# LPD-EPFL-ML/X-MAP

Measured on AMD Instinct MI355X. Metric: item_sim_pairs_per_s, higher is better.
Workload: dtype f64

## Files before the change

x-map_amd/csrc/api.hip:

```cpp
#include <math.h>
#include <stdlib.h>
#include <vector>

#include "common.h"

namespace xmap {

struct Pool {
    std::vector<void *> ptrs;
    void release() {
        for (void *p : ptrs) (void)hipFree(p);
        ptrs.clear();
    }
};

}

using namespace xmap;

struct xmap_ctx {
    int device = 0;
    hipStream_t st = nullptr;
    Pool p_ratings, p_sim, p_ext, p_gen, p_rows;
    xmap_ratings R;
    bool have_ratings = false;
    bool plain_exact = true;
    bool have_sim = false;
    xmap_sim S;
    double *u_avg = nullptr, *u_norm = nullptr, *info = nullptr;
    int64_t n_kept = 0, n_eval = 0, n_contrib = 0;
    int64_t half_contrib = 0;
    bool have_ext = false;
    int top_k = 0;
    xmap_ext_tables T;
    xmap_path_units Un;
    int32_t *n_cand = nullptr, *top_end = nullptr;
    double *top_val = nullptr;
    int64_t n_out = 0, n_paths = 0;
    double *acc = nullptr, *hacc = nullptr;
    int32_t *touched = nullptr, *htouched = nullptr;
    int64_t acc_slots = 0, acc_len = 0, hacc_rows = 0, hacc_len = 0;
    int32_t n_slots = 0;
    int32_t fast_div = 0;
    bool have_gen = false;
    int32_t *g_user = nullptr, *g_item = nullptr;
    double *g_rating = nullptr;
    int64_t *g_time = nullptr;
    int64_t n_rows = 0, n_target_rows = 0;
};

namespace xmap {

template <typename T>
static int dalloc(Pool &pool, T **out, size_t n, hipStream_t st, bool zero = false) {
    void *p = nullptr;
    const size_t bytes = sizeof(T) * (n ? n : 1);
    XM_HIP(hipMalloc(&p, bytes));
    pool.ptrs.push_back(p);
    if (zero) XM_HIP(hipMemsetAsync(p, 0, bytes, st));
    *out = (T *)p;
    return XMAP_OK;
}
#define XM_TRY(call) do { int rc_ = (call); if (rc_) return rc_; } while (0)
#define XM_ALLOC(pool, ptr, n) XM_TRY(dalloc(pool, &(ptr), (size_t)(n), c->st))
#define XM_ALLOCZ(pool, ptr, n) XM_TRY(dalloc(pool, &(ptr), (size_t)(n), c->st, true))

template <typename T>
static int h2d(Pool &pool, T **out, const T *host, size_t n, hipStream_t st) {
    XM_TRY(dalloc(pool, out, n, st));
    if (n) XM_HIP(hipMemcpyAsync(*out, host, sizeof(T) * n, hipMemcpyHostToDevice, st));
    return XMAP_OK;
}
template <typename T>
static int d2h(T *host, const T *dev, size_t n, hipStream_t st) {
    if (n) XM_HIP(hipMemcpyAsync(host, dev, sizeof(T) * n, hipMemcpyDeviceToHost, st));
    return XMAP_OK;
}

static int reverse_list(xmap_ctx *c, int mode, const uint8_t *bb, const int64_t *attach_ptr, const void *thr, int32_t *long_rows,
                        uint8_t *eflag, int32_t *counted ,
                        const int64_t **rptr, const int32_t **ridx, const double **rval, const uint8_t **rflag) {
    const int I = c->R.n_items, k = c->top_k;
    int32_t *rcnt = counted;
    int64_t *ptr;
    XM_ALLOCZ(c->p_ext, ptr, I + 1);
    if (!counted) {
        XM_ALLOCZ(c->p_ext, rcnt, I);
        XM_TRY(xmap_reverse_count(c->st, &c->S, mode, k, bb, c->T.cls, c->T.kcnt, c->T.kcol, c->T.kval, c->R.suffix_cls,
                                  c->R.contains_mask, c->R.flags, attach_ptr, thr, long_rows, eflag, rcnt, 0, I));
    }
    int64_t n = 0;
    XM_TRY(xmap_exclusive_scan_i32_to_i64(c->st, rcnt, ptr, I, &n));
    int32_t *idx;
    double *val;
    uint8_t *flag;
    XM_ALLOC(c->p_ext, idx, n);
    XM_ALLOC(c->p_ext, val, 3 * (size_t)(n ? n : 1));
    XM_ALLOCZ(c->p_ext, flag, n);
    XM_TRY(xmap_reverse_fill(c->st, &c->S, mode, k, bb, c->T.cls, c->T.kcnt, c->T.kcol, c->T.kval, c->R.suffix_cls,
                             c->R.contains_mask, c->R.flags, attach_ptr, thr, long_rows, eflag, ptr, idx, val, flag, 0, I));
    *rptr = ptr; *ridx = idx; *rval = val; *rflag = flag;
    return XMAP_OK;
}

static int ensure_rows(xmap_ctx *c, int64_t slots, int64_t len, int64_t hrows) {
    if (c->acc == nullptr || c->acc_slots < slots || c->acc_len != len || c->hacc_rows < hrows) {
        c->p_rows.release();
        c->acc = nullptr; c->hacc = nullptr;
        XM_ALLOCZ(c->p_rows, c->acc, (size_t)slots * len * 4);
        XM_ALLOC(c->p_rows, c->touched, (size_t)slots * len);
        if (hrows) {
            XM_ALLOCZ(c->p_rows, c->hacc, (size_t)hrows * len * 4);
            XM_ALLOC(c->p_rows, c->htouched, (size_t)hrows * len);
        }
        c->acc_slots = slots; c->acc_len = len; c->hacc_rows = hrows;
    }
    return XMAP_OK;
}

static int run_enumeration(xmap_ctx *c, int64_t xs_cap, int64_t *xs_off, int32_t *xs_end, double *xs_val) {
    const int I = c->R.n_items;
    xmap_path_rows Rw;
    Rw.n_slots = c->n_slots; Rw.acc = c->acc; Rw.touched = c->touched; Rw.hacc = c->hacc; Rw.htouched = c->htouched;
    xmap_path_out O;
    O.n_cand = c->n_cand; O.top_end = c->top_end; O.top_val = c->top_val;
    O.xs_cap = xs_cap; O.xs_off = xs_off; O.xs_end = xs_end; O.xs_val = xs_val;
    XM_HIP(hipMemsetAsync(c->n_cand, 0, sizeof(int32_t) * (size_t)I, c->st));
    XM_HIP(hipMemsetAsync(c->top_end, 0xff, sizeof(int32_t) * (size_t)I * XMAP_TOPC, c->st));
    XM_HIP(hipMemsetAsync(c->top_val, 0, sizeof(double) * (size_t)I * XMAP_TOPC, c->st));
    int64_t *d_cnt;
    XM_ALLOCZ(c->p_ext, d_cnt, 8);
    int64_t h_cnt[8] = {0, 0, 0, 0, 0, 0, 0, 0};
    int rc;
    if (c->T.n_nb > 0) {
        rc = xmap_extend_cols(c->st, &c->T, &c->Un, &Rw, &O, c->fast_div, d_cnt, h_cnt);
    } else {
        rc = xmap_extend_paths(c->st, I, c->top_k, c->T.cls, c->T.kcnt, c->T.kcol, c->T.kval, c->T.flags, c->T.att_ptr, c->T.att_idx,
                               c->T.att_val, c->T.src_ptr, c->T.src_idx, c->T.src_val, c->T.src_flag, c->T.rnn_ptr, c->T.rnn_idx,
                               c->T.rnn_val, c->Un.n_units, c->Un.unit_start, c->Un.unit_c, c->Un.unit_G, c->Un.unit_row,
                               c->Un.unit_nt, c->Un.n_heavy, c->Un.heavy_unit0, c->n_slots, c->acc, c->touched, c->hacc, c->htouched,
                               c->n_cand, c->top_end, c->top_val, xs_cap, xs_off, xs_end, xs_val, d_cnt, h_cnt);
    }
    if (rc && rc != XMAP_ERR_CAPACITY) {
        c->p_rows.release();
        c->acc = nullptr;
    }
    c->n_out = h_cnt[0]; c->n_paths = h_cnt[1];
    return rc;
// ... 272 lines not shown
        dir = dir_c; midX = mid_c;
        XM_TRY(xmap_mid_rows_place(c->st, I, k, cls, kcnt, kcol, kval, c->R.flags, T.att_ptr, T.att_idx, T.att_val, T.src_ptr, T.src_idx,
                                   T.src_val, T.src_flag, (int32_t)n_nb, nb_list, nb_id, dir_ptr, rec_ptr, dir, midX));
        T.dir = dir; T.midX = midX; T.dir_ptr = dir_ptr;
    }
    int64_t len = I;
    if (n_nb > 0) {
        int32_t *mark, *urank, *uitem;
        int64_t *rank, n_ends = 0;
        XM_ALLOC(c->p_ext, mark, I); XM_ALLOC(c->p_ext, rank, I + 1); XM_ALLOC(c->p_ext, urank, I); XM_ALLOC(c->p_ext, uitem, I);
        XM_TRY(xmap_end_universe(c->st, &T, mark, rank, urank, uitem, &n_ends));
        XM_TRY(xmap_end_order(c->st, I, k, (int32_t)n_nb, nb_list, kcnt, kcol, (int32_t)n_ends, urank, uitem));
        T.n_ends = (int32_t)n_ends; T.urank = urank; T.uitem = uitem;
        len = n_ends > 0 ? n_ends : 1;
    }
    int32_t resident = 0;
    XM_TRY(xmap_extend_cols_slots(&resident));
    int64_t n_slots = resident;
    const int64_t slot_cap = ((int64_t)24 << 30) / (36 * len);
    if (n_slots > slot_cap) n_slots = slot_cap > 4 ? slot_cap : 4;
    const int64_t max_rows = ((int64_t)16 << 30) / (36 * len) > 2 ? ((int64_t)16 << 30) / (36 * len) : 2;
    const int64_t cap_units = (int64_t)I + max_rows;
    int32_t *unit_start, *unit_c, *unit_G, *unit_row, *unit_nt, *heavy_unit0;
    XM_ALLOC(c->p_ext, unit_start, cap_units); XM_ALLOC(c->p_ext, unit_c, cap_units); XM_ALLOC(c->p_ext, unit_G, cap_units);
    XM_ALLOC(c->p_ext, unit_row, cap_units); XM_ALLOC(c->p_ext, heavy_unit0, I);
    int64_t hp[5];
    XM_TRY(xmap_path_plan(c->st, I, P, 0, I, 0, 8192, max_rows, cap_units, unit_start, unit_c, unit_G, unit_row, heavy_unit0, hp));
    XM_ALLOCZ(c->p_ext, unit_nt, hp[0]);
    xmap_path_units &Un = c->Un;
    Un.n_units = (int32_t)hp[0]; Un.unit_start = unit_start; Un.unit_c = unit_c; Un.unit_G = unit_G; Un.unit_row = unit_row;
    Un.unit_nt = unit_nt; Un.n_heavy = (int32_t)hp[1]; Un.heavy_unit0 = heavy_unit0;
    if (n_slots > hp[0]) n_slots = hp[0] > 4 ? hp[0] : 4;
    c->n_slots = (int32_t)n_slots;
    XM_TRY(ensure_rows(c, n_slots, len, hp[2]));
    XM_TRY(run_enumeration(c, 0, nullptr, nullptr, nullptr));
    c->have_ext = true;
    if (n_out) *n_out = c->n_out;
    if (n_paths) *n_paths = c->n_paths;
    return XMAP_OK;
}

int xmap_ctx_ext_download(xmap_ctx *c, int32_t *n_cand, int32_t *top_end, double *top_val) {
    XM_ARG(c && c->have_ext);
    XM_HIP(hipSetDevice(c->device));
    const size_t I = (size_t)c->R.n_items;
    if (n_cand) XM_TRY(d2h(n_cand, (const int32_t *)c->n_cand, I, c->st));
    if (top_end) XM_TRY(d2h(top_end, (const int32_t *)c->top_end, I * XMAP_TOPC, c->st));
    if (top_val) XM_TRY(d2h(top_val, (const double *)c->top_val, I * XMAP_TOPC, c->st));
    XM_HIP(hipStreamSynchronize(c->st));
    return XMAP_OK;
}

int xmap_ctx_ext_lists(xmap_ctx *c, int64_t *xs_off, int32_t *xs_end, double *xs_val) {
    XM_ARG(c && c->have_ext && xs_off && (c->n_out == 0 || (xs_end && xs_val)));
    XM_HIP(hipSetDevice(c->device));
    const int I = c->R.n_items;
    if (I == 0) return XMAP_OK;
    const int64_t cap = c->n_out > 0 ? c->n_out : 1;
    Pool tmp;
    struct Guard { Pool &p; ~Guard() { p.release(); } } guard{tmp};
    int64_t *d_off;
    int32_t *d_end;
    double *d_val;
    XM_TRY(dalloc(tmp, &d_off, (size_t)I, c->st, true));
    XM_TRY(dalloc(tmp, &d_end, (size_t)cap, c->st));
    XM_TRY(dalloc(tmp, &d_val, (size_t)cap, c->st));
    XM_TRY(run_enumeration(c, cap, d_off, d_end, d_val));
// ... 66 lines not shown
```

x-map_amd/csrc/paths.h:

```cpp
#pragma once
#include "common.h"

namespace xmap {

struct PathArgs {
    int I, k;
    const uint8_t *cls;
    const int *kcnt;
    const int *kcol;
    const double *kval;
    const uint8_t *flags;
    const long long *att_ptr; const int *att_idx; const double *att_val;
    const long long *src_ptr; const int *src_idx; const double *src_val; const uint8_t *src_flag;
    const long long *rnn_ptr; const int *rnn_idx; const double *rnn_val;
    int n_units;
    const int *unit_start; const int *unit_c; const int *unit_G; const int *unit_row; int *unit_nt;
    int n_slots;
    double *acc; int *touched;
    double *hacc; int *htouched;
    int *n_cand; int *top_end; double *top_val;
    long long xs_cap; long long *xs_off; int *xs_end; double *xs_val;
    unsigned long long *counters;
    int U; const int *urank; const int *uitem;
    long long row_stride;
// ... 85 lines not shown
            unsigned long long ok = __shfl_xor(bk, m, 64);
            int oe = __shfl_xor(be, m, 64);
            double ov = __shfl_xor(bv, m, 64);
            int oh = __shfl_xor((int)have, m, 64);
            if (oh && (!have || ok > bk || (ok == bk && oe < be))) { bk = ok; be = oe; bv = ov; have = true; }
        }
        pk = bk; pe = be;
        if (lane == 0) { top_end[r] = be; top_val[r] = bv; }
    }
}

constexpr int FIN_CAP = 128;
struct FinBuf { double v[FIN_CAP + 64]; int e[FIN_CAP + 64]; double ov[XMAP_TOPC]; int oe[XMAP_TOPC]; };

__device__ __forceinline__ unsigned long long xsim_key(double v) { return (unsigned long long)__double_as_longlong(fabs(v)); }

__device__ __forceinline__ bool fin_list_offset(const PathArgs &A, int nt, int start, unsigned long long &off) {
    off = 0;
    if (!(A.xs_cap > 0 && nt > 0)) return false;
    if (lane_id() == 0) off = atomicAdd(&A.counters[3], (unsigned long long)nt);
    off = ((unsigned long long)(unsigned)rl32((int)(off >> 32), 0) << 32) | (unsigned)rl32((int)(off & 0xffffffffull), 0);
    const bool full = (long long)(off + nt) <= A.xs_cap;
    if (lane_id() == 0) A.xs_off[start] = full ? (long long)off : -1;
    return full;
}

__device__ __forceinline__ int fin_cut(FinBuf &F, int nbuf, int *out_e, double *out_v) {
    volatile double *bv = F.v;
    volatile int *be = F.e;
    select_topc(nbuf, [&](int b, int &e, double &v) { e = be[b]; v = bv[b]; }, out_e, out_v);
    return nbuf < XMAP_TOPC ? nbuf : XMAP_TOPC;
}

__device__ __forceinline__ int finalize_slice(const PathArgs &A, FinBuf &F, double *acc, const int *touched, int nt,
                                              unsigned long long off, bool full, int w, int NW, int gs = 1, int mem = 0) {
    const int lane = lane_id();
    volatile double *bv = F.v;
    volatile int *be = F.e;
    int nbuf = 0;
    unsigned long long thr = 0;
    for (int b0 = 64 * w; b0 < nt; b0 += 64 * NW) {
        const int b = b0 + lane;
        const bool act = b < nt;
        int e = 0;
        double v = 0.0;
        unsigned long long key = 0;
        if (act) {
            e = touched[b];
            double *a = acc + ((size_t)e * gs + mem) * 4;
            v = 1.0 * (a[0] + a[1]) / (a[2] + a[3]);
            a[0] = 0.0; a[1] = 0.0; a[2] = 0.0; a[3] = 0.0;
            key = xsim_key(v);
            if (full) { A.xs_end[off + b] = A.uitem ? A.uitem[e] : e; A.xs_val[off + b] = v; }
        }
        const bool q = act && key >= thr;
        const unsigned long long m = __ballot(q);
        if (q) { const int p = nbuf + __popcll(m & lanemask_lt()); bv[p] = v; be[p] = A.uitem ? A.uitem[e] : e; }
        nbuf += __popcll(m);
        if (nbuf > FIN_CAP) {
            const int ns = fin_cut(F, nbuf, F.oe, F.ov);
            int te = 0;
            double tv = 0.0;
            if (lane < ns) { te = ((volatile int *)F.oe)[lane]; tv = ((volatile double *)F.ov)[lane]; }
            if (lane < ns) { be[lane] = te; bv[lane] = tv; }
            nbuf = ns;
            thr = (ns == XMAP_TOPC) ? xsim_key(rld(tv, XMAP_TOPC - 1)) : 0ull;
        }
    }
    return fin_cut(F, nbuf, F.oe, F.ov);
}

__device__ __forceinline__ int finalize_start(const PathArgs &A, FinBuf &F, double *acc, const int *touched, int nt, int start,
                                              int gs = 1, int mem = 0) {
    const int lane = lane_id();
    if (lane == 0) A.n_cand[start] = nt;
    unsigned long long off;
    const bool full = fin_list_offset(A, nt, start, off);
    const int ns = finalize_slice(A, F, acc, touched, nt, off, full, 0, 1, gs, mem);
    if (lane < ns) {
        A.top_end[(size_t)start * XMAP_TOPC + lane] = ((volatile int *)F.oe)[lane];
        A.top_val[(size_t)start * XMAP_TOPC + lane] = ((volatile double *)F.ov)[lane];
    }
    return nt;
}

struct MidX { double sm2, sm3, sm4, f2, f3, f4, mu; int xid; int pad; };
struct MidDir { int x; int ne; int cnt; int pad; long long off; };

template <int SRC>
__device__ __forceinline__ double quad_bcast(double v) {
    constexpr int CTRL = SRC | (SRC << 2) | (SRC << 4) | (SRC << 6);
    const long long b = __double_as_longlong(v);
    const int lo = __builtin_amdgcn_update_dpp(0, (int)(b & 0xffffffffll), CTRL, 0xf, 0xf, true);
    const int hi = __builtin_amdgcn_update_dpp(0, (int)(b >> 32), CTRL, 0xf, 0xf, true);
    return __longlong_as_double(((long long)hi << 32) | (unsigned int)lo);
}

struct ColEnd { double sm, mu, f; int u; int pad; };
struct Path2Args {
    PathArgs P;
    const ColEnd *cend;
    const int *nb_id; const int *nb_list; int n_nb;
    const MidX *midX; const MidDir *dir; const long long *dir_ptr; const int *ng;
};

template <class ACC>
__device__ __forceinline__ void head_S(const PathArgs &A, ACC &W, int xp, bool has_e1, Carry e1) {
    const int lane = lane_id();
    const int nb = A.kcnt[(size_t)xp * 2];
    for (int q = 0; q < nb; q++) {
        const size_t o = ((size_t)xp * 2) * A.k + q;
        const int t = A.kcol[o];
        if (!(A.flags[t] & 2)) continue;
        const Carry c2 = has_e1 ? add_edge(e1, A.kval[o * 3], A.kval[o * 3 + 1], A.kval[o * 3 + 2])
                                : first_edge(A.kval[o * 3], A.kval[o * 3 + 1], A.kval[o * 3 + 2]);
        const long long s0 = A.src_ptr[t], s1 = A.src_ptr[t + 1];
        for (long long base = s0; base < s1; base += 64) {
            const long long p = base + lane;
            const bool act = (p < s1) && (A.src_flag[p] & 1);
            int s = 0;
            Carry c = c2;
            if (act) {
                s = A.src_idx[p];
                c = add_edge(c2, A.src_val[p * 3], A.src_val[p * 3 + 1], A.src_val[p * 3 + 2]);
            }
            W.add(act, s, c);
        }
    }
}

int merge_heavy(hipStream_t st, const PathArgs &A, int n_heavy, const int *heavy_unit0);

}
```

x-map_amd/csrc/paths4.hip:

```cpp
#include "paths.h"

namespace xmap {

__device__ __forceinline__ double div_mid(double a, double b) {
    double y = __builtin_amdgcn_rcp(b);
    double e = __builtin_fma(-b, y, 1.0);
    y = __builtin_fma(y, e, y);
    e = __builtin_fma(-b, y, 1.0);
    y = __builtin_fma(y, e, y);
    const double q = a * y;
    const double r = __builtin_fma(-b, q, a);
    return __builtin_fma(r, y, q);
}

__device__ __forceinline__ void acc2(double &hi, double &lo, double x) {
    const double s = hi + x;
    const double bb = s - hi;
    lo += (hi - (s - bb)) + (x - bb);
    hi = s;
}

template <int CTRL>
__device__ __forceinline__ double quad_swap(double v) {
    const long long b = __double_as_longlong(v);
    const int lo = __builtin_amdgcn_update_dpp(0, (int)(b & 0xffffffffll), CTRL, 0xf, 0xf, true);
    const int hi = __builtin_amdgcn_update_dpp(0, (int)(b >> 32), CTRL, 0xf, 0xf, true);
    return __longlong_as_double(((long long)hi << 32) | (unsigned int)lo);
}


constexpr int Q_CAP = 64;
struct QLds {
    double bsm[Q_CAP + 1], bc[Q_CAP + 1], bmu[Q_CAP + 1];
    double hd[3][64];
    uint4 ep[128];
};

struct QAcc {
    double *acc; int *touched;
    const int *urank;
    int nt;
    unsigned long long paths;
    unsigned long long updates;
    __device__ __forceinline__ void add(bool active, int end, Carry p) {
        bool first = false;
        int u = 0;
        if (active) {
            u = urank[end];
            const double sp = (p.mu != 0.0) ? 1.0 * p.sm / p.mu : 0.0;
            double *a = acc + (size_t)u * 4;
            double s_hi = a[0], s_lo = a[1], c_hi = a[2], c_lo = a[3];
            first = (c_hi == 0.0);
            acc2(s_hi, s_lo, sp * p.c);
            acc2(c_hi, c_lo, p.c);
            a[0] = s_hi; a[1] = s_lo; a[2] = c_hi; a[3] = c_lo;
        }
        const unsigned long long m = __ballot(first);
        if (first) touched[nt + __popcll(m & lanemask_lt())] = u;
        nt += __popcll(m);
        const int na = __popcll(__ballot(active));
        paths += na;
        updates += na;
    }
};

__device__ double g_zero_entry[4] = {0.0, 0.0, 0.0, 0.0};
constexpr int END_HOME = 1 << 30;

template <bool FASTDIV>
__device__ __forceinline__ void heads_Q(const Path2Args &B, QAcc &W, int start, long long h0, long long nH, int self, int xlo, int xhi,
                                        bool fresh) {
    __shared__ QLds stageq[4];
    const PathArgs &A = B.P;
    QLds &L = stageq[threadIdx.x >> 6];
    const int lane = lane_id();
    const int k = A.k;
    const int INF = 0x7fffffff;
    const long long h = h0 + lane;
    const bool hv = h < nH;
    double sm1 = 0.0, mu1 = 0.0, f1 = 1.0;
    long long dpos = 0, dend = 0;
    if (hv) {
        int xp = start;
        if (h >= self) {
            const long long rp = A.rnn_ptr[start] + (h - self);
            xp = A.rnn_idx[rp];
            const double sv = A.rnn_val[rp * 3], mu = A.rnn_val[rp * 3 + 1];
            sm1 = sv * mu; mu1 = mu; f1 = A.rnn_val[rp * 3 + 2];
        }
        const int xpid = B.nb_id[xp];
        dpos = B.dir_ptr[xpid];
        dend = B.dir_ptr[xpid + 1];
        if (xlo > 0) {
// ... 120 lines not shown
                    acc2(a_ch, a_cl, c);
                };
                int it = 0;
                for (; it + 1 < steps; it += 2) {
                    const int ra = (it << sh) + slice, rb = ra + ns;
                    const int rbc = rb < fill ? rb : Q_CAP;
                    const double s0 = L.bsm[ra], c0 = L.bc[ra], u0 = L.bmu[ra];
                    const double s1 = L.bsm[rbc], c1 = L.bc[rbc], u1 = L.bmu[rbc];
                    asm volatile("" :: "v"(s0), "v"(c0), "v"(u0), "v"(s1), "v"(c1), "v"(u1));
                    step(s0, c0, u0);
                    step(s1, c1, u1);
                }
                if (it < steps) {
                    const int ra = (it << sh) + slice;
                    const int rc_ = ra < fill ? ra : Q_CAP;
                    step(L.bsm[rc_], L.bc[rc_], L.bmu[rc_]);
                }
                if (sh >= 1) {
                    const double o_sh = quad_swap<0xB1>(a_sh), o_sl = quad_swap<0xB1>(a_sl);
                    const double o_ch = quad_swap<0xB1>(a_ch), o_cl = quad_swap<0xB1>(a_cl);
                    acc2(a_sh, a_sl, o_sh); a_sl += o_sl;
                    acc2(a_ch, a_cl, o_ch); a_cl += o_cl;
                }
                if (sh == 2) {
                    const double o_sh = quad_swap<0x4E>(a_sh), o_sl = quad_swap<0x4E>(a_sl);
                    const double o_ch = quad_swap<0x4E>(a_ch), o_cl = quad_swap<0x4E>(a_cl);
                    acc2(a_sh, a_sl, o_sh); a_sl += o_sl;
                    acc2(a_ch, a_cl, o_ch); a_cl += o_cl;
                }
                asm volatile("" :: "v"(h0_), "v"(l0_), "v"(h1_), "v"(l1_) : "memory");
                bool first = false;
                if (fl_) {
                    first = (h1_ == 0.0);
                    acc2(h0_, l0_, a_sh); l0_ += a_sl;
                    acc2(h1_, l1_, a_ch); l1_ += a_cl;
                }
                if (sh >= 1) {
                    const double p_h = quad_swap<0xB1>(h1_), p_l = quad_swap<0xB1>(l1_);
                    double *dst = a + (slice == 0 ? 0 : 2);
                    const double v0 = slice == 0 ? h0_ : p_h, v1 = slice == 0 ? l0_ : p_l;
                    if (ok && slice <= 1) { dst[0] = v0; dst[1] = v1; }
                } else if (fl_) {
                    a[0] = h0_; a[1] = l0_; a[2] = h1_; a[3] = l1_;
                }
                const unsigned long long fm = __ballot(first);
                if (first) W.touched[W.nt + __popcll(fm & lanemask_lt())] = eu;
                W.nt += __popcll(fm);
                W.paths += (unsigned long long)fill * (unsigned long long)nact;
                W.updates += (unsigned long long)nact;
                if (!pm) break;
                assign();
                m0 = recp[my_rec];
            }
        }
        if (mine) {
            dpos++;
            cur.x = INF;
            if (dpos < dend) { cur = B.dir[dpos]; if (cur.x >= xhi) cur.x = INF; }
        }
    }
}


constexpr int P_WAVES = 5;
template <bool FASTDIV>
__global__ __launch_bounds__(256) __attribute__((amdgpu_waves_per_eu(P_WAVES, P_WAVES))) void k_paths4(Path2Args B) {
// ... 28 lines not shown
        const long long nH = self + (r1 - r0);
        const long long nbatch = (nH + 63) / 64;
        const int RX = (nbatch > 0) ? (int)((G + nbatch - 1) / nbatch) : 1;
        const int n_nb = B.n_nb;
        long long ent = (role_t ? 1 : 0) + nH;
        for (long long bt = 0; bt < nbatch; bt++)
            for (int rx = 0; rx < RX; rx++) {
                if (G == 1 || ent % G == c) {
                    const int xlo = (rx == 0) ? 0 : B.nb_list[(long long)rx * n_nb / RX];
                    const int xhi = (rx == RX - 1) ? 0x7fffffff : B.nb_list[(long long)(rx + 1) * n_nb / RX];
                    heads_Q<FASTDIV>(B, W, start, bt * 64, nH, self, xlo, xhi, bt == 0);
                }
                ent++;
            }
        ent = 0;
        if (role_t) {
            if (G == 1 || ent % G == c) {
                Carry none; none.sm = 0; none.mu = 0; none.c = 0;
                through_t(A, W, start, false, none);
            }
            ent++;
        }
        for (long long h = 0; h < nH; h++) {
            if (G == 1 || ent % G == c) {
                const bool has_e1 = h >= self;
                const int xp = has_e1 ? A.rnn_idx[r0 + h - self] : start;
                Carry e1; e1.sm = 0; e1.mu = 0; e1.c = 1.0;
                if (has_e1) e1 = first_edge(A.rnn_val[(r0 + h - self) * 3], A.rnn_val[(r0 + h - self) * 3 + 1],
                                            A.rnn_val[(r0 + h - self) * 3 + 2]);
                head_S(A, W, xp, has_e1, e1);
            }
            ent++;
        }
        if (row < 0) cand_total += finalize_start(A, fin[threadIdx.x >> 6], W.acc, W.touched, W.nt, start);
        else if (lane == 0) A.unit_nt[unit] = W.nt;
    }
    if (lane == 0) {
        atomicAdd(&A.counters[0], cand_total);
        atomicAdd(&A.counters[1], W.paths);
        atomicAdd(&A.counters[4], W.updates);
    }
}

__global__ __launch_bounds__(256) void k_edge_ranges(long long n, const double *sim, const int *mutu, int *bad) {
    const long long p = (long long)blockIdx.x * blockDim.x + threadIdx.x;
    if (p >= n) return;
    const double m = (double)mutu[p], sm = fabs(sim[p] * m);
    const bool ok = (m >= 1.0) && (sm == 0.0 || (sm > 0x1p-400 && sm < 0x1p400));
    if (!ok) atomicOr(bad, 1);
}

__global__ __launch_bounds__(256) void k_col_home(int n_nb, int k, const int *nb_list, const int *kcnt, const int *kcol, int *home) {
    const long long t = (long long)blockIdx.x * blockDim.x + threadIdx.x;
    if (t >= (long long)n_nb * (k + 1)) return;
    const int xid = (int)(t / (k + 1)), idx = (int)(t % (k + 1));
    const int x = nb_list[xid];
    int e = -1;
    if (idx == 0) e = x;
    else if (idx - 1 < kcnt[(size_t)x * 2 + 1]) e = kcol[((size_t)x * 2 + 1) * k + (idx - 1)];
    if (e >= 0) atomicMin(&home[e], x);
}

__global__ __launch_bounds__(256) void k_col_ends(int n_nb, int k, const int *nb_list, const int *kcnt, const int *kcol, const double *kval,
                                                  const int *urank, const int *home, ColEnd *cend) {
    const long long t = (long long)blockIdx.x * blockDim.x + threadIdx.x;
    if (t >= (long long)n_nb * (k + 1)) return;
    const int xid = (int)(t / (k + 1)), idx = (int)(t % (k + 1));
// ... 6 lines not shown
        const size_t o = ((size_t)x * 2 + 1) * k + (idx - 1);
        const double v = kval[o * 3], m = kval[o * 3 + 1];
        e.sm = v * m; e.mu = m; e.f = kval[o * 3 + 2];
        item = kcol[o];
    }
    if (item >= 0) e.u = urank[item] | (home[item] == x ? END_HOME : 0);
    cend[t] = e;
}

__global__ __launch_bounds__(256) void k_mark_ends(int I, int k, const uint8_t *cls, const int *kcnt, const int *kcol, long long n_src,
                                                   const int *src_idx, long long n_att, const int *att_idx, int *mark) {
    const long long t = (long long)blockIdx.x * blockDim.x + threadIdx.x;
    if (t < n_src) mark[src_idx[t]] = 1;
    if (t < n_att) mark[att_idx[t]] = 1;
    if (t < (long long)I * k) {
        const int x = (int)(t / k), q = (int)(t % k);
        if (cls[x] == 2) {
            if (q == 0) mark[x] = 1;
            if (q < kcnt[(size_t)x * 2 + 1]) mark[kcol[((size_t)x * 2 + 1) * k + q]] = 1;
        }
    }
}
__global__ __launch_bounds__(256) void k_end_ranks(int I, const int *mark, const long long *rank64, int *urank, int *uitem) {
    const int i = blockIdx.x * blockDim.x + threadIdx.x;
    if (i >= I) return;
    const int r = (int)rank64[i];
    urank[i] = mark[i] ? r : -1;
    if (mark[i]) uitem[r] = i;
}

constexpr int MERGE_WAVES = 16;
constexpr int MERGE_GROUP = 12;

__device__ __forceinline__ void merge_row(double *acc_d, int *touched_d, int *s_nt, double *acc_s, const int *touched_s, int nt_s) {
    const int lane = lane_id(), w = threadIdx.x >> 6;
    const int half = (lane & 1) * 2;
    for (int b0 = 32 * w; b0 < nt_s; b0 += 32 * MERGE_WAVES) {
        const int b = b0 + (lane >> 1);
        bool first = false;
        int e = 0;
        if (b < nt_s) {
            e = touched_s[b];
            double *s = acc_s + (size_t)e * 4 + half, *d = acc_d + (size_t)e * 4 + half;
            double hi = d[0], lo = d[1];
            first = half == 2 && hi == 0.0;
            dd_add(hi, lo, s[0]); dd_add(hi, lo, s[1]);
            d[0] = hi; d[1] = lo;
            s[0] = 0.0; s[1] = 0.0;
        }
        const unsigned long long m = __ballot(first);
        int base = 0;
        if (lane == 0 && m) base = atomicAdd(s_nt, __popcll(m));
        base = rl32(base, 0);
        if (first) touched_d[base + __popcll(m & lanemask_lt())] = e;
    }
    __syncthreads();
}

__global__ __launch_bounds__(64 * MERGE_WAVES) void k_merge_groups(PathArgs A, int n_heavy, const int *heavy_unit0) {
    __shared__ int s_nt;
    const int h = blockIdx.x;
    if (h >= n_heavy) return;
    const int u0 = heavy_unit0[h];
    const int G = A.unit_G[u0], r0 = A.unit_row[u0];
    if (G <= MERGE_GROUP) return;
    for (int g = blockIdx.y; g * MERGE_GROUP < G; g += gridDim.y) {
        const int b = g * MERGE_GROUP;
        const int e = (b + MERGE_GROUP) < G ? (b + MERGE_GROUP) : G;
        if (threadIdx.x == 0) s_nt = A.unit_nt[u0 + b];
        __syncthreads();
        for (int c = b + 1; c < e; c++)
            merge_row(A.hacc + (size_t)(r0 + b) * A.U * 4, A.htouched + (size_t)(r0 + b) * A.U, &s_nt,
                      A.hacc + (size_t)(r0 + c) * A.U * 4, A.htouched + (size_t)(r0 + c) * A.U, A.unit_nt[u0 + c]);
        if (threadIdx.x == 0) A.unit_nt[u0 + b] = s_nt;
        __syncthreads();
    }
}

__global__ __launch_bounds__(64 * MERGE_WAVES) void k_merge(PathArgs A, int n_heavy, const int *heavy_unit0) {
    __shared__ FinBuf fin[MERGE_WAVES];
    __shared__ int s_nt, s_ns[MERGE_WAVES], s_full;
    __shared__ unsigned long long s_off;
    const int h = blockIdx.x;
    if (h >= n_heavy) return;
    const int lane = lane_id(), w = threadIdx.x >> 6;
    const int u0 = heavy_unit0[h];
    const int start = A.unit_start[u0], G = A.unit_G[u0], r0 = A.unit_row[u0];
    double *acc0 = A.hacc + (size_t)r0 * A.U * 4;
    int *touched0 = A.htouched + (size_t)r0 * A.U;
    if (threadIdx.x == 0) s_nt = A.unit_nt[u0];
    __syncthreads();
    const int stride = G > MERGE_GROUP ? MERGE_GROUP : 1;
    for (int c = stride; c < G; c += stride)
        merge_row(acc0, touched0, &s_nt, A.hacc + (size_t)(r0 + c) * A.U * 4, A.htouched + (size_t)(r0 + c) * A.U,
                  A.unit_nt[u0 + c]);
    const int nt = s_nt;
    if (w == 0) {
        if (lane == 0) A.n_cand[start] = nt;
        unsigned long long off;
        const bool full = fin_list_offset(A, nt, start, off);
        if (lane == 0) { s_off = off; s_full = full ? 1 : 0; }
    }
    __syncthreads();
    const int ns = finalize_slice(A, fin[w], acc0, touched0, nt, s_off, s_full != 0, w, MERGE_WAVES);
    if (lane == 0) s_ns[w] = ns;
    __syncthreads();
    if (w == 0) {
        volatile double *bv = fin[0].v;
        volatile int *be = fin[0].e;
        int nbuf = 0;
        for (int o = 0; o < MERGE_WAVES; o++) {
            const int n = s_ns[o];
            int te = 0;
            double tv = 0.0;
            if (lane < n) { te = ((volatile int *)fin[o].oe)[lane]; tv = ((volatile double *)fin[o].ov)[lane]; }
            if (lane < n) { be[nbuf + lane] = te; bv[nbuf + lane] = tv; }
            nbuf += n;
        }
        fin_cut(fin[0], nbuf, A.top_end + (size_t)start * XMAP_TOPC, A.top_val + (size_t)start * XMAP_TOPC);
        if (lane == 0) atomicAdd(&A.counters[0], (unsigned long long)nt);
    }
}

int merge_heavy(hipStream_t st, const PathArgs &A, int n_heavy, const int *heavy_unit0) {
    k_merge_groups<<<dim3((unsigned)n_heavy, 16), dim3(64 * MERGE_WAVES), 0, st>>>(A, n_heavy, heavy_unit0);
    XM_LAUNCH_CHECK();
    k_merge<<<dim3((unsigned)n_heavy), dim3(64 * MERGE_WAVES), 0, st>>>(A, n_heavy, heavy_unit0);
    XM_LAUNCH_CHECK();
    return XMAP_OK;
}

}

using namespace xmap;

extern "C" {

int xmap_edge_ranges(void *stream, const xmap_sim *S, int32_t *h_fast_ok) {
    XM_SCOPE(stream);
    XM_ARG(S && h_fast_ok);
    *h_fast_ok = 1;
    if (S->n_items == 0) return XMAP_OK;
    hipStream_t st = (hipStream_t)stream;
    long long n = 0;
    XM_HIP(hipMemcpyAsync(&n, S->row_ptr + S->n_items, sizeof(long long), hipMemcpyDeviceToHost, st));
    XM_HIP(hipStreamSynchronize(st));
    if (n == 0) return XMAP_OK;
    if (S->frac) { *h_fast_ok = 0; return XMAP_OK; }
    int *bad = nullptr;
    XM_HIP(xm_malloc_async((void **)&bad, sizeof(int), st));
    XM_HIP(hipMemsetAsync(bad, 0, sizeof(int), st));
    k_edge_ranges<<<dim3((unsigned)((n + 255) / 256)), dim3(256), 0, st>>>(n, S->sim, S->mutu, bad);
    XM_LAUNCH_CHECK();
    int h = 0;
    XM_HIP(hipMemcpyAsync(&h, bad, sizeof(int), hipMemcpyDeviceToHost, st));
    XM_HIP(hipStreamSynchronize(st));
    XM_HIP(xm_free_async(bad, st));
    *h_fast_ok = h ? 0 : 1;
    return XMAP_OK;
}
// ... 58 lines not shown
        A.rnn_ptr = (const long long *)T->rnn_ptr; A.rnn_idx = T->rnn_idx; A.rnn_val = T->rnn_val;
        A.n_units = Un->n_units; A.unit_start = Un->unit_start; A.unit_c = Un->unit_c; A.unit_G = Un->unit_G;
        A.unit_row = Un->unit_row; A.unit_nt = Un->unit_nt;
        A.acc = R->acc; A.touched = R->touched; A.hacc = R->hacc; A.htouched = R->htouched;
        A.n_cand = O->n_cand; A.top_end = O->top_end; A.top_val = O->top_val;
        A.xs_cap = O->xs_cap; A.xs_off = (long long *)O->xs_off; A.xs_end = O->xs_end; A.xs_val = O->xs_val;
        A.counters = (unsigned long long *)d_counters;
        A.U = T->n_ends; A.urank = T->urank; A.uitem = T->uitem;
        A.n_slots = R->n_slots < Un->n_units ? R->n_slots : Un->n_units;
        B.nb_id = T->nb_id; B.nb_list = T->nb_list; B.n_nb = T->n_nb; B.midX = (const MidX *)T->midX; B.dir = (const MidDir *)T->dir;
        B.dir_ptr = (const long long *)T->dir_ptr; B.ng = nullptr;
        A.row_stride = T->n_ends;
        ColEnd *cend = nullptr;
        int *home = nullptr;
        if (T->n_nb > 0) {
            const long long n = (long long)T->n_nb * (T->top_k + 1);
            XM_HIP(xm_malloc_async((void **)&cend, sizeof(ColEnd) * (size_t)n, st));
            XM_HIP(xm_malloc_async((void **)&home, sizeof(int) * (size_t)T->n_items, st));
            XM_HIP(hipMemsetAsync(home, 0x7f, sizeof(int) * (size_t)T->n_items, st));
            const dim3 cgrid((unsigned)((n + 255) / 256));
            k_col_home<<<cgrid, dim3(256), 0, st>>>(T->n_nb, T->top_k, T->nb_list, T->kcnt, T->kcol, home);
            XM_LAUNCH_CHECK();
            k_col_ends<<<cgrid, dim3(256), 0, st>>>(T->n_nb, T->top_k, T->nb_list, T->kcnt, T->kcol, T->kval, T->urank, home, cend);
            XM_LAUNCH_CHECK();
            XM_HIP(xm_free_async(home, st));
        }
        B.cend = cend;
        const dim3 grid((unsigned)((A.n_slots + 3) / 4)), block(256);
        if (fast_div) k_paths4<true><<<grid, block, 0, st>>>(B);
        else k_paths4<false><<<grid, block, 0, st>>>(B);
        XM_LAUNCH_CHECK();
        if (cend) XM_HIP(xm_free_async(cend, st));
        if (Un->n_heavy > 0) {
            const int rc = merge_heavy(st, A, Un->n_heavy, Un->heavy_unit0);
            if (rc) return rc;
        }
    }
    if (h_counters) {
        XM_HIP(hipMemcpyAsync(h_counters, d_counters, 8 * sizeof(int64_t), hipMemcpyDeviceToHost, st));
        XM_HIP(hipStreamSynchronize(st));
        if (O->xs_cap > 0 && h_counters[0] > O->xs_cap) {
            set_error("candidate buffer too small: need %lld entries, have %lld", (long long)h_counters[0], (long long)O->xs_cap);
            return XMAP_ERR_CAPACITY;
        }
    }
    return XMAP_OK;
}
}
```

x-map_amd/csrc/stage_b.hip:

```cpp
#include "paths.h"
#include <stdlib.h>

namespace xmap {

__global__ __launch_bounds__(256) void k_bridge_flags(int I, const long long *row_ptr, const int *col,
                                                      const int *prefix_cls, uint8_t *bb) {
    int i = blockIdx.x * 4 + (threadIdx.x >> 6);
    if (i >= I) return;
    int lane = lane_id();
    long long lo = row_ptr[i], hi = row_ptr[i + 1];
    int pi = prefix_cls[i];
    int found = 0;
    for (long long b = lo; b < hi && !found; b += 64) {
        long long p = b + lane;
        int f = (p < hi) && (prefix_cls[col[p]] != pi);
        found = __ballot(f) != 0ull;
    }
    if (lane == 0) bb[i] = (uint8_t)found;
}

constexpr int K_THREADS = 256;
constexpr int K_CH = 2048;
constexpr int K_CH_SMALL = 512;
constexpr int K_WIN = 1024;
// ... 1296 lines not shown
    XM_ARG(n_units == 0 || (unit_start && unit_c && unit_G && unit_row && unit_nt));
    XM_ARG(n_heavy == 0 || (heavy_unit0 && hacc && htouched));
    XM_ARG(xs_cap == 0 || (xs_off && xs_end && xs_val));
    hipStream_t st = (hipStream_t)stream;
    XM_HIP(hipMemsetAsync(d_counters, 0, 4 * sizeof(int64_t), st));
    if (n_units > 0) {
        PathArgs A;
        A.I = n_items; A.k = top_k;
        A.cls = cls; A.kcnt = kcnt; A.kcol = kcol; A.kval = kval; A.flags = flags;
        A.att_ptr = (const long long *)att_ptr; A.att_idx = att_idx; A.att_val = att_val;
        A.src_ptr = (const long long *)src_ptr; A.src_idx = src_idx; A.src_val = src_val; A.src_flag = src_flag;
        A.rnn_ptr = (const long long *)rnn_ptr; A.rnn_idx = rnn_idx; A.rnn_val = rnn_val;
        A.n_units = n_units; A.unit_start = unit_start; A.unit_c = unit_c; A.unit_G = unit_G; A.unit_row = unit_row;
        A.unit_nt = unit_nt;
        A.n_slots = n_slots; A.acc = acc; A.touched = touched; A.hacc = hacc; A.htouched = htouched;
        A.n_cand = n_cand; A.top_end = top_end; A.top_val = top_val;
        A.xs_cap = xs_cap; A.xs_off = (long long *)xs_off; A.xs_end = xs_end; A.xs_val = xs_val;
        A.counters = (unsigned long long *)d_counters;
        A.U = n_items; A.urank = nullptr; A.uitem = nullptr; A.row_stride = n_items;
        int slots = n_slots < n_units ? n_slots : n_units;
        A.n_slots = slots;
#ifdef XMAP_CROSSCHECK
        if (mid) {
            Path2Args B = *mid;
            B.P = A;
            k_paths2<<<dim3((unsigned)((slots + 3) / 4)), dim3(256), 0, st>>>(B);
        } else
#endif
        {
            k_paths<<<dim3((unsigned)((slots + 3) / 4)), dim3(256), 0, st>>>(A);
        }
        XM_LAUNCH_CHECK();
        if (n_heavy > 0) {
            const int rc = merge_heavy(st, A, n_heavy, heavy_unit0);
            if (rc) return rc;
        }
    }
    if (h_counters) {
        XM_HIP(hipMemcpyAsync(h_counters, d_counters, 4 * sizeof(int64_t), hipMemcpyDeviceToHost, st));
        XM_HIP(hipStreamSynchronize(st));
        if (xs_cap > 0 && h_counters[0] > xs_cap) {
            set_error("candidate buffer too small: need %lld entries, have %lld", (long long)h_counters[0],
                      (long long)xs_cap);
            return XMAP_ERR_CAPACITY;
        }
    }
    return XMAP_OK;
}

int xmap_extend_paths(void *stream, int32_t n_items, int top_k, const uint8_t *cls, const int32_t *kcnt,
                      const int32_t *kcol, const double *kval, const uint8_t *flags, const int64_t *att_ptr,
                      const int32_t *att_idx, const double *att_val, const int64_t *src_ptr, const int32_t *src_idx,
                      const double *src_val, const uint8_t *src_flag, const int64_t *rnn_ptr, const int32_t *rnn_idx,
                      const double *rnn_val, int32_t n_units, const int32_t *unit_start, const int32_t *unit_c,
                      const int32_t *unit_G, const int32_t *unit_row, int32_t *unit_nt, int32_t n_heavy,
                      const int32_t *heavy_unit0, int32_t n_slots, double *acc, int32_t *touched, double *hacc,
                      int32_t *htouched, int32_t *n_cand, int32_t *top_end, double *top_val, int64_t xs_cap,
                      int64_t *xs_off, int32_t *xs_end, double *xs_val, int64_t *d_counters, int64_t *h_counters) {
    return extend_paths_impl(nullptr, stream, n_items, top_k, cls, kcnt, kcol, kval, flags, att_ptr, att_idx, att_val, src_ptr, src_idx, src_val, src_flag, rnn_ptr, rnn_idx, rnn_val, n_units, unit_start, unit_c, unit_G, unit_row, unit_nt, n_heavy, heavy_unit0, n_slots, acc, touched, hacc, htouched, n_cand, top_end, top_val, xs_cap, xs_off, xs_end, xs_val, d_counters, h_counters);
}

#ifdef XMAP_CROSSCHECK
int xmap_extend_paths2(void *stream, int32_t n_items, int top_k, const uint8_t *cls, const int32_t *kcnt,
                      const int32_t *kcol, const double *kval, const uint8_t *flags, const int64_t *att_ptr,
                      const int32_t *att_idx, const double *att_val, const int64_t *src_ptr, const int32_t *src_idx,
                      const double *src_val, const uint8_t *src_flag, const int64_t *rnn_ptr, const int32_t *rnn_idx,
                      const double *rnn_val, int32_t n_units, const int32_t *unit_start, const int32_t *unit_c,
// ... 200 lines not shown
```

Before: 23.04 billion.

## Use lazy half-zeroing of accumulator rows and lane-pair split updates

In the paths4 path, accumulator entries are no longer fully zeroed at finalize. Only the count half (a[2],a[3]) is cleared, and the sum half is reset lazily when a lane sees an empty count. The per-path add now spreads each 4-double accumulator update across two lanes, with DPP exchanging emptiness between them, and merge kernels are templated to follow the same convention. The aim is to cut store traffic on finalize and merge and to spread accumulator memory accesses across lanes. The cost is two shuffle rounds per add, and correctness now depends on every path honouring the lazy-reset invariant, which is why rows are reallocated when the mode changes.

Result: no change. 23.06 billion, median of 3 (+0.1%).

```diff
diff --git a/x-map_amd/csrc/api.hip b/x-map_amd/csrc/api.hip
--- a/x-map_amd/csrc/api.hip
+++ b/x-map_amd/csrc/api.hip
@@ -40,6 +40,7 @@
     double *acc = nullptr, *hacc = nullptr;
     int32_t *touched = nullptr, *htouched = nullptr;
     int64_t acc_slots = 0, acc_len = 0, hacc_rows = 0, hacc_len = 0;
+    bool acc_wrows = false;
     int32_t n_slots = 0;
     int32_t fast_div = 0;
     bool have_gen = false;
@@ -103,8 +104,8 @@
     return XMAP_OK;
 }
 
-static int ensure_rows(xmap_ctx *c, int64_t slots, int64_t len, int64_t hrows) {
-    if (c->acc == nullptr || c->acc_slots < slots || c->acc_len != len || c->hacc_rows < hrows) {
+static int ensure_rows(xmap_ctx *c, int64_t slots, int64_t len, int64_t hrows, bool wrows) {
+    if (c->acc == nullptr || c->acc_slots < slots || c->acc_len != len || c->hacc_rows < hrows || c->acc_wrows != wrows) {
         c->p_rows.release();
         c->acc = nullptr; c->hacc = nullptr;
         XM_ALLOCZ(c->p_rows, c->acc, (size_t)slots * len * 4);
@@ -113,7 +114,7 @@
             XM_ALLOCZ(c->p_rows, c->hacc, (size_t)hrows * len * 4);
             XM_ALLOC(c->p_rows, c->htouched, (size_t)hrows * len);
         }
-        c->acc_slots = slots; c->acc_len = len; c->hacc_rows = hrows;
+        c->acc_slots = slots; c->acc_len = len; c->hacc_rows = hrows; c->acc_wrows = wrows;
     }
     return XMAP_OK;
 }
@@ -452,7 +453,7 @@
     Un.unit_nt = unit_nt; Un.n_heavy = (int32_t)hp[1]; Un.heavy_unit0 = heavy_unit0;
     if (n_slots > hp[0]) n_slots = hp[0] > 4 ? hp[0] : 4;
     c->n_slots = (int32_t)n_slots;
-    XM_TRY(ensure_rows(c, n_slots, len, hp[2]));
+    XM_TRY(ensure_rows(c, n_slots, len, hp[2], n_nb > 0));
     XM_TRY(run_enumeration(c, 0, nullptr, nullptr, nullptr));
     c->have_ext = true;
     if (n_out) *n_out = c->n_out;
diff --git a/x-map_amd/csrc/paths.h b/x-map_amd/csrc/paths.h
--- a/x-map_amd/csrc/paths.h
+++ b/x-map_amd/csrc/paths.h
@@ -141,6 +141,7 @@
     return nbuf < XMAP_TOPC ? nbuf : XMAP_TOPC;
 }
 
+template <bool WROWS = false>
 __device__ __forceinline__ int finalize_slice(const PathArgs &A, FinBuf &F, double *acc, const int *touched, int nt,
                                               unsigned long long off, bool full, int w, int NW, int gs = 1, int mem = 0) {
     const int lane = lane_id();
@@ -158,7 +159,13 @@
             e = touched[b];
             double *a = acc + ((size_t)e * gs + mem) * 4;
             v = 1.0 * (a[0] + a[1]) / (a[2] + a[3]);
-            a[0] = 0.0; a[1] = 0.0; a[2] = 0.0; a[3] = 0.0;
+            if (WROWS) {
+                double z0 = 0.0, z1 = 0.0;
+                asm volatile("" : "+v"(z0), "+v"(z1));
+                a[2] = z0; a[3] = z1;
+            } else {
+                a[0] = 0.0; a[1] = 0.0; a[2] = 0.0; a[3] = 0.0;
+            }
             key = xsim_key(v);
             if (full) { A.xs_end[off + b] = A.uitem ? A.uitem[e] : e; A.xs_val[off + b] = v; }
         }
@@ -179,13 +186,14 @@
     return fin_cut(F, nbuf, F.oe, F.ov);
 }
 
+template <bool WROWS = false>
 __device__ __forceinline__ int finalize_start(const PathArgs &A, FinBuf &F, double *acc, const int *touched, int nt, int start,
                                               int gs = 1, int mem = 0) {
     const int lane = lane_id();
     if (lane == 0) A.n_cand[start] = nt;
     unsigned long long off;
     const bool full = fin_list_offset(A, nt, start, off);
-    const int ns = finalize_slice(A, F, acc, touched, nt, off, full, 0, 1, gs, mem);
+    const int ns = finalize_slice<WROWS>(A, F, acc, touched, nt, off, full, 0, 1, gs, mem);
     if (lane < ns) {
         A.top_end[(size_t)start * XMAP_TOPC + lane] = ((volatile int *)F.oe)[lane];
         A.top_val[(size_t)start * XMAP_TOPC + lane] = ((volatile double *)F.ov)[lane];
@@ -238,6 +246,6 @@
     }
 }
 
-int merge_heavy(hipStream_t st, const PathArgs &A, int n_heavy, const int *heavy_unit0);
-
-}
+int merge_heavy(hipStream_t st, const PathArgs &A, int n_heavy, const int *heavy_unit0, bool wrows);
+
+}
diff --git a/x-map_amd/csrc/paths4.hip b/x-map_amd/csrc/paths4.hip
--- a/x-map_amd/csrc/paths4.hip
+++ b/x-map_amd/csrc/paths4.hip
@@ -43,22 +43,39 @@
     unsigned long long paths;
     unsigned long long updates;
     __device__ __forceinline__ void add(bool active, int end, Carry p) {
-        bool first = false;
+        const int lane = lane_id();
         int u = 0;
+        double x_s = 0.0, x_c = 0.0;
         if (active) {
             u = urank[end];
             const double sp = (p.mu != 0.0) ? 1.0 * p.sm / p.mu : 0.0;
-            double *a = acc + (size_t)u * 4;
-            double s_hi = a[0], s_lo = a[1], c_hi = a[2], c_lo = a[3];
-            first = (c_hi == 0.0);
-            acc2(s_hi, s_lo, sp * p.c);
-            acc2(c_hi, c_lo, p.c);
-            a[0] = s_hi; a[1] = s_lo; a[2] = c_hi; a[3] = c_lo;
-        }
-        const unsigned long long m = __ballot(first);
-        if (first) touched[nt + __popcll(m & lanemask_lt())] = u;
-        nt += __popcll(m);
-        const int na = __popcll(__ballot(active));
+            x_s = sp * p.c; x_c = p.c;
+        }
+        const unsigned long long am = __ballot(active);
+        const int half = (lane & 1) * 2;
+        for (int h = 0; h < 2; h++) {
+            const unsigned int hm = (unsigned int)(am >> (32 * h));
+            if (!hm) continue;
+            const int src = 32 * h + (lane >> 1);
+            const int uu = __shfl(u, src, 64);
+            const double xs = __shfl(x_s, src, 64), xc = __shfl(x_c, src, 64);
+            const double x = half ? xc : xs;
+            bool first = false;
+            if ((hm >> (lane >> 1)) & 1) {
+                double *a = acc + (size_t)uu * 4 + half;
+                double hi = a[0], lo = a[1];
+                const bool empty = hi == 0.0;
+                first = half == 2 && empty;
+                const int pair_empty = __builtin_amdgcn_update_dpp(0, (int)empty, 0xB1, 0xf, 0xf, true);
+                if (half == 0 && pair_empty) { hi = 0.0; lo = 0.0; }
+                acc2(hi, lo, x);
+                a[0] = hi; a[1] = lo;
+            }
+            const unsigned long long m = __ballot(first);
+            if (first) touched[nt + __popcll(m & lanemask_lt())] = uu;
+            nt += __popcll(m);
+        }
+        const int na = __popcll(am);
         paths += na;
         updates += na;
     }
@@ -245,6 +262,7 @@
                 bool first = false;
                 if (fl_) {
                     first = (h1_ == 0.0);
+                    if (first) { h0_ = 0.0; l0_ = 0.0; }
                     acc2(h0_, l0_, a_sh); l0_ += a_sl;
                     acc2(h1_, l1_, a_ch); l1_ += a_cl;
                 }
@@ -339,7 +357,7 @@
             }
             ent++;
         }
-        if (row < 0) cand_total += finalize_start(A, fin[threadIdx.x >> 6], W.acc, W.touched, W.nt, start);
+        if (row < 0) cand_total += finalize_start<true>(A, fin[threadIdx.x >> 6], W.acc, W.touched, W.nt, start);
         else if (lane == 0) A.unit_nt[unit] = W.nt;
     }
     if (lane == 0) {
@@ -412,6 +430,7 @@
 constexpr int MERGE_WAVES = 16;
 constexpr int MERGE_GROUP = 12;
 
+template <bool WROWS>
 __device__ __forceinline__ void merge_row(double *acc_d, int *touched_d, int *s_nt, double *acc_s, const int *touched_s, int nt_s) {
     const int lane = lane_id(), w = threadIdx.x >> 6;
     const int half = (lane & 1) * 2;
@@ -423,10 +442,15 @@
             e = touched_s[b];
             double *s = acc_s + (size_t)e * 4 + half, *d = acc_d + (size_t)e * 4 + half;
             double hi = d[0], lo = d[1];
-            first = half == 2 && hi == 0.0;
+            const bool empty = hi == 0.0;
+            first = half == 2 && empty;
+            if (WROWS) {
+                const int pair_empty = __builtin_amdgcn_update_dpp(0, (int)empty, 0xB1, 0xf, 0xf, true);
+                if (half == 0 && pair_empty) { hi = 0.0; lo = 0.0; }
+            }
             dd_add(hi, lo, s[0]); dd_add(hi, lo, s[1]);
             d[0] = hi; d[1] = lo;
-            s[0] = 0.0; s[1] = 0.0;
+            if (!WROWS || half == 2) { s[0] = 0.0; s[1] = 0.0; }
         }
         const unsigned long long m = __ballot(first);
         int base = 0;
@@ -437,6 +461,7 @@
     __syncthreads();
 }
 
+template <bool WROWS>
 __global__ __launch_bounds__(64 * MERGE_WAVES) void k_merge_groups(PathArgs A, int n_heavy, const int *heavy_unit0) {
     __shared__ int s_nt;
     const int h = blockIdx.x;
@@ -450,13 +475,14 @@
         if (threadIdx.x == 0) s_nt = A.unit_nt[u0 + b];
         __syncthreads();
         for (int c = b + 1; c < e; c++)
-            merge_row(A.hacc + (size_t)(r0 + b) * A.U * 4, A.htouched + (size_t)(r0 + b) * A.U, &s_nt,
+            merge_row<WROWS>(A.hacc + (size_t)(r0 + b) * A.U * 4, A.htouched + (size_t)(r0 + b) * A.U, &s_nt,
                       A.hacc + (size_t)(r0 + c) * A.U * 4, A.htouched + (size_t)(r0 + c) * A.U, A.unit_nt[u0 + c]);
         if (threadIdx.x == 0) A.unit_nt[u0 + b] = s_nt;
         __syncthreads();
     }
 }
 
+template <bool WROWS>
 __global__ __launch_bounds__(64 * MERGE_WAVES) void k_merge(PathArgs A, int n_heavy, const int *heavy_unit0) {
     __shared__ FinBuf fin[MERGE_WAVES];
     __shared__ int s_nt, s_ns[MERGE_WAVES], s_full;
@@ -472,7 +498,7 @@
     __syncthreads();
     const int stride = G > MERGE_GROUP ? MERGE_GROUP : 1;
     for (int c = stride; c < G; c += stride)
-        merge_row(acc0, touched0, &s_nt, A.hacc + (size_t)(r0 + c) * A.U * 4, A.htouched + (size_t)(r0 + c) * A.U,
+        merge_row<WROWS>(acc0, touched0, &s_nt, A.hacc + (size_t)(r0 + c) * A.U * 4, A.htouched + (size_t)(r0 + c) * A.U,
                   A.unit_nt[u0 + c]);
     const int nt = s_nt;
     if (w == 0) {
@@ -482,7 +508,7 @@
         if (lane == 0) { s_off = off; s_full = full ? 1 : 0; }
     }
     __syncthreads();
-    const int ns = finalize_slice(A, fin[w], acc0, touched0, nt, s_off, s_full != 0, w, MERGE_WAVES);
+    const int ns = finalize_slice<WROWS>(A, fin[w], acc0, touched0, nt, s_off, s_full != 0, w, MERGE_WAVES);
     if (lane == 0) s_ns[w] = ns;
     __syncthreads();
     if (w == 0) {
@@ -502,10 +528,13 @@
     }
 }
 
-int merge_heavy(hipStream_t st, const PathArgs &A, int n_heavy, const int *heavy_unit0) {
-    k_merge_groups<<<dim3((unsigned)n_heavy, 16), dim3(64 * MERGE_WAVES), 0, st>>>(A, n_heavy, heavy_unit0);
+int merge_heavy(hipStream_t st, const PathArgs &A, int n_heavy, const int *heavy_unit0, bool wrows) {
+    const dim3 ggrid((unsigned)n_heavy, 16), mgrid((unsigned)n_heavy), block(64 * MERGE_WAVES);
+    if (wrows) k_merge_groups<true><<<ggrid, block, 0, st>>>(A, n_heavy, heavy_unit0);
+    else k_merge_groups<false><<<ggrid, block, 0, st>>>(A, n_heavy, heavy_unit0);
     XM_LAUNCH_CHECK();
-    k_merge<<<dim3((unsigned)n_heavy), dim3(64 * MERGE_WAVES), 0, st>>>(A, n_heavy, heavy_unit0);
+    if (wrows) k_merge<true><<<mgrid, block, 0, st>>>(A, n_heavy, heavy_unit0);
+    else k_merge<false><<<mgrid, block, 0, st>>>(A, n_heavy, heavy_unit0);
     XM_LAUNCH_CHECK();
     return XMAP_OK;
 }
@@ -630,7 +659,7 @@
         XM_LAUNCH_CHECK();
         if (cend) XM_HIP(xm_free_async(cend, st));
         if (Un->n_heavy > 0) {
-            const int rc = merge_heavy(st, A, Un->n_heavy, Un->heavy_unit0);
+            const int rc = merge_heavy(st, A, Un->n_heavy, Un->heavy_unit0, true);
             if (rc) return rc;
         }
     }
diff --git a/x-map_amd/csrc/stage_b.hip b/x-map_amd/csrc/stage_b.hip
--- a/x-map_amd/csrc/stage_b.hip
+++ b/x-map_amd/csrc/stage_b.hip
@@ -1352,7 +1352,7 @@
         }
         XM_LAUNCH_CHECK();
         if (n_heavy > 0) {
-            const int rc = merge_heavy(st, A, n_heavy, heavy_unit0);
+            const int rc = merge_heavy(st, A, n_heavy, heavy_unit0, false);
             if (rc) return rc;
         }
     }
```
